# filrg/attackFL

Hardware: AMD Instinct MI355X
Metric: FL rounds/sec (whole node) + test-acc, TransformerModel/ICU, 8 clients (higher is better)
Workload: dtype bf16; 1 GPU; model=TransformerModel, global_batch=1024, seq_len=1, parallelism=fl8-clients-over-1-ranks, clients=8, local_epochs=5, rows_per_client=12000-15000, mode=fedavg, trainer=fused

## Files before the change

csrc/kernels/tf2.hip:

```cpp
#include "common.h"
#include "kernels.h"
#include "tf_common.h"
#include "fused_common.h"
#include "onchip.h"

using namespace tf;

namespace t2 {

using namespace oc;



constexpr int LDDN = 24 * 2, LDVO = LD64 + 16;
constexpr int B_IMG_D = 0;
constexpr int B_IMG_V = B_IMG_D + 64 * LDDN;
constexpr int B_IMG_O = B_IMG_V + 64 * LDVO;
constexpr int B_IMG_F1 = B_IMG_O + 64 * LDVO;
constexpr int B_IMG_F2 = B_IMG_F1 + 16 * LD64;
constexpr int B_H0 = B_IMG_F2 + 64 * LD32;
constexpr int B_A = B_H0 + 16384;
constexpr int B_X1N = B_A + 16384;
constexpr int B_DF3 = B_X1N + 16384;
constexpr int B_DO = B_DF3 + 16384;
constexpr int B_DV = B_DO + 16384;
constexpr int B_DZ0 = B_DV + 16384;
constexpr int B_XIN = B_DZ0 + 16384;
constexpr int B_F2 = B_XIN + 4096;
constexpr int B_DF0 = B_F2 + 4096;
constexpr int B_NVEC = 648;
constexpr int B_VEC = B_DF0 + 4096;
constexpr int B_CS = B_VEC + B_NVEC * 4;
constexpr int B_NLN = 6 * 64;
constexpr int B_DBL = B_CS;
constexpr int B_DBL_BYTES = B_NLN * 8;
static_assert(B_DBL_BYTES >= B_NVEC * 4, "DBL covers CS");
constexpr int B_MISC = B_DBL + B_DBL_BYTES;
constexpr int B_CNT_A = B_MISC + 32;
constexpr int B_CNT_B = B_MISC + 36;
constexpr int B_CNT_C = B_MISC + 40;
constexpr int B_TOTAL = B_MISC + 64;
enum { VS_DB = 0, VS_VB, VS_OB, VS_G1, VS_B1, VS_F2B, VS_G2, VS_B2, VS_G3, VS_B3 };
constexpr int VS_F1B = 640;

#ifndef TF2_HLD1
#define TF2_HLD1 (LD128 + 16)
#endif
#ifndef TF2_HLD2
#define TF2_HLD2 (LD64 + 16)
#endif
constexpr int HLD1 = TF2_HLD1, HLD2 = TF2_HLD2;
constexpr int H_IMG_W1 = 0;
constexpr int H_IMG_W2 = H_IMG_W1 + 64 * HLD1;
constexpr int H_CAT = H_IMG_W2 + 32 * HLD2;
constexpr int H_A1 = H_CAT + 32768;
constexpr int H_DZ1 = H_A1 + 16384;
constexpr int H_DZ2 = H_DZ1 + 16384;
constexpr int H_NVEC = 132;
constexpr int H_VEC = H_DZ2 + 8192;
constexpr int H_PART = H_VEC + H_NVEC * 4;
constexpr int H_LOSS = H_PART + 8 * H_NVEC * 4;
constexpr int H_TOTAL = H_LOSS + 64;
enum { HV_B1 = 0, HV_B2 = 64, HV_WO = 96, HV_BO = 128 };

constexpr int SMEM_CORE = B_TOTAL > H_TOTAL ? B_TOTAL : H_TOTAL;
#ifdef TF2_STAMPS
constexpr int ST_OFF = SMEM_CORE, ST_N = 16;
constexpr int SMEM = ST_OFF + ST_N * 8;
#else
constexpr int SMEM = SMEM_CORE;
#endif
static_assert(SMEM <= 160 * 1024, "LDS budget");

constexpr int MOM_SLOTS = 11;
constexpr long WS_MOM = 0;
constexpr long MOM_WG_BYTES = (long)MOM_SLOTS * NTH * 16;
constexpr int CMP_SLOTS = 1;
constexpr long BR_UNITS = (long)CMP_SLOTS * NTH * 16;
constexpr long BR_SMALL = BR_UNITS + 8L * 12 * 64 * 16;
constexpr long BR_WG_BYTES = BR_SMALL + 4L * 9 * 64 * 16;
constexpr long WS_BYTES = WS_MOM + MOM_WG_BYTES + 2 * BR_WG_BYTES;

__device__ __forceinline__ void ln_colsum(uchar* smem, int k, const float (&x)[16], int lane) {
  float s;
  const int f = colsum64(x, lane, s);
  lds_addq(smem + B_DBL, 64 * k + f, s);
}
__host__ __device__ constexpr int ln_seg(int k) { return k < 2 ? VS_G1 + k : VS_G2 + (k - 2); }
static_assert(ln_seg(0) == VS_G1 && ln_seg(1) == VS_B1 && ln_seg(2) == VS_G2 && ln_seg(3) == VS_B2 &&
              ln_seg(4) == VS_G3 && ln_seg(5) == VS_B3, "DBL order");

__device__ __forceinline__ uint32_t mask16(uint32_t key, uint32_t layer, int r, int g, uint32_t thr) {
  uint32_t m = 0;
#pragma unroll
  for (int t = 0; t < 4; ++t) {
#pragma unroll
    for (int h = 0; h < 2; ++h) {
      const uint32_t x = hash3(key, layer, (uint32_t)r, (uint32_t)(8 * t + 2 * g + h));
      m |= ((x & 0xFFFFu) >= thr ? 1u : 0u) << (4 * t + 2 * h);
      m |= ((x >> 16) >= thr ? 1u : 0u) << (4 * t + 2 * h + 1);
    }
  }
  return m;
}


#ifdef TF2_STAMPS
struct Stamp {
  bool on = false;
  int who = 0;
  uchar* smem = nullptr;
  __device__ __forceinline__ void operator()(int id, int tid) {
    if (!on) return;
    const uint64_t now = __builtin_amdgcn_s_memrealtime();
    if (tid == who) {
      LDS_AS uint64_t* t = (LDS_AS uint64_t*)(smem + ST_OFF);
      t[id] += now - t[ST_N - 1];
      t[ST_N - 1] = now;
    }
  }
};
#else
struct Stamp {
  __device__ __forceinline__ void operator()(int, int) {}
};
#endif

enum { ABL_U3 = 1, ABL_UADAM = 2, ABL_UDW = 4, ABL_COLSUM = 8, ABL_HEADUPD = 16, ABL_U1 = 32 };
#if defined(TF2_STAMPS) && defined(TF2_ABL)
#define ABL(K, b) ((TF2_ABL & (b)) != 0)
#else
#define ABL(K, b) false
#endif



#ifndef TF2_NO_PRIO
__device__ __forceinline__ void prio_hi() { __builtin_amdgcn_s_setprio(2); }
__device__ __forceinline__ void prio_lo() { __builtin_amdgcn_s_setprio(0); }
#else
__device__ __forceinline__ void prio_hi() {}
__device__ __forceinline__ void prio_lo() {}
#endif

template <int BR>
struct BrK {
  static constexpr BrOff o = BR == 0 ? OV : OL;
  static constexpr int din = BR == 0 ? D_V : D_L;
  static constexpr int xoff = BR == 0 ? 0 : D_V;
  static constexpr Mat MV{o.inproj_w + 128 * 64, 64, 64, B_IMG_V, LDVO};
  static constexpr Mat MO{o.out_w, 64, 64, B_IMG_O, LDVO};
  static __device__ __forceinline__ Mat vo(bool lo) {
    return Mat{lo ? MV.off : MO.off, 64, 64, lo ? B_IMG_V : B_IMG_O, LDVO};
  }
  static __device__ __forceinline__ int vec_param(int e) {
    if (e >= VS_F1B) return e - VS_F1B < FF ? o.ff0_b + (e - VS_F1B) : -1;
    const int s = e >> 6, i = e & 63;
    const int b = s == 0 ? o.dense_b : s == 1 ? o.inproj_b + 128 : s == 2 ? o.out_b : s == 3 ? o.ln1_w
                : s == 4 ? o.ln1_b : s == 5 ? o.ff3_b : s == 6 ? o.ln2_w : s == 7 ? o.ln2_b : s == 8 ? o.bn_w : o.bn_b;
    return b + i;
  }
};

struct Saved {
  uint32_t xh1[8], xh2[8], gp[8];
  float rstd1, rstd2;
  uint32_t m1, m2, matt;
  float gk[4];
};
__device__ __forceinline__ void save16(uint32_t (&d)[8], const float (&x)[16]) {
#pragma unroll
  for (int k = 0; k < 8; ++k) d[k] = pk2(x[2 * k], x[2 * k + 1]);
}
__device__ __forceinline__ void load16(float (&x)[16], const uint32_t (&d)[8]) {
#pragma unroll
  for (int k = 0; k < 8; ++k) {
    x[2 * k] = __uint_as_float(d[k] << 16);
    x[2 * k + 1] = __uint_as_float(d[k] & 0xFFFF0000u);
  }
}

constexpr int NCMP = 2;
struct BrState {
  VS cmp[NCMP];
  float dst[NCMP];
};
static_assert(B_NVEC <= NCMP * NTH, "compact entries");

template <int BR>
__device__ __forceinline__ void br_masks(uint32_t key, int r, int g, uint32_t& mk0, uint32_t& mk1) {
  const uint32_t ha = hash3(key, 8 * BR + L_ATT, r, 0), hb = hash3(key, 8 * BR + L_ATT, r, 1);
  const uint32_t matt = ((ha & 0xFFFFu) >= THR_P01 ? 1u : 0u) | ((ha >> 16) >= THR_P01 ? 2u : 0u) |
                        ((hb & 0xFFFFu) >= THR_P01 ? 4u : 0u) | ((hb >> 16) >= THR_P01 ? 8u : 0u);
  const uint32_t m1 = mask16(key, 8 * BR + L_D1, r, g, THR_P01), m2 = mask16(key, 8 * BR + L_D2, r, g, THR_P01);
  uint32_t kf = 0u;
  if (g < 2) {
    const uint32_t hd[2] = {hash3(key, 8 * BR + L_DF, r, 2 * g), hash3(key, 8 * BR + L_DF, r, 2 * g + 1)};
#pragma unroll
    for (int i = 0; i < 4; ++i) {
      const uint32_t u = (hd[i >> 1] >> ((i & 1) << 4)) & 0xFFFFu;
      kf |= (4 * g + i < FF && u >= THR_P01 ? 1u : 0u) << i;
    }
  }
  mk0 = m1 | (m2 << 16);
  mk1 = matt | (kf << 4);
}

template <int BR>
__device__ __forceinline__ void br_forward(uchar* smem, const float (&xin)[4], uint32_t mk0, uint32_t mk1, Saved& sv,
                                           u32x4 (&outp)[2], int lane, int wave) {
  using B = BrK<BR>;
  opq(lane, wave);
  const int g = lane >> 4, r = 16 * wave + (lane & 15);
  const uchar* vg = lane_vec(smem + B_VEC, g);
  st4<TK16>(smem + B_XIN, r, g, xin);
  float h0[16];
  sb();
  {
    const s4v bx = bfrag4(xin);
    f4v acc[4];
#pragma unroll
    for (int T = 0; T < 4; ++T)
      acc[T] = mma16(*(const LDS_AS s4v*)(smem + B_IMG_D + (16 * T + (lane & 15)) * LDDN + 8 * (lane >> 4)), bx, Z4);
    float bd[16], gp[16];
    vec16g(bd, vg + VS_DB * 256);
#pragma unroll
    for (int t = 0; t < 4; ++t)
#pragma unroll
      for (int i = 0; i < 4; i += 2) {
        gf2v g2;
        const gf2v y = gelu2(gf2v{acc[t][i] + bd[4 * t + i], acc[t][i + 1] + bd[4 * t + i + 1]}, g2);
        h0[4 * t + i] = y[0];
        h0[4 * t + i + 1] = y[1];
        gp[4 * t + i] = g2[0];
        gp[4 * t + i + 1] = g2[1];
      }
    save16(sv.gp, gp);
#pragma unroll
    for (int t = 0; t < 4; ++t) st4<TK64>(smem + B_H0, r, 4 * t + g, h0 + 4 * t);
  }
  float a[16];
  sb();
  {
    const s8v b0 = bfrag(h0, 0), b1 = bfrag(h0, 1);
    f4v acc[4];
#pragma unroll
    for (int T = 0; T < 4; ++T) {
      acc[T] = mma(wfrag(smem + B_IMG_V, LDVO, T, 0, lane), b0, Z4);
      acc[T] = mma(wfrag(smem + B_IMG_V, LDVO, T, 1, lane), b1, acc[T]);
    }
    sv.matt = mk1 & 0xFu;
    float bv[16];
    vec16g(bv, vg + VS_VB * 256);
#pragma unroll
    for (int t = 0; t < 4; ++t) {
      const float m = keepf(INV_K01, sv.matt, t);
#pragma unroll
      for (int i = 0; i < 4; ++i) a[4 * t + i] = (acc[t][i] + bv[4 * t + i]) * m;
    }
#pragma unroll
    for (int t = 0; t < 4; ++t) st4<TK64>(smem + B_A, r, 4 * t + g, a + 4 * t);
  }
  float x1n[16];
  sb();
  {
    const s8v b0 = bfrag(a, 0), b1 = bfrag(a, 1);
    f4v acc[4];
#pragma unroll
    for (int T = 0; T < 4; ++T) {
      acc[T] = mma(wfrag(smem + B_IMG_O, LDVO, T, 0, lane), b0, Z4);
      acc[T] = mma(wfrag(smem + B_IMG_O, LDVO, T, 1, lane), b1, acc[T]);
    }
    sv.m1 = mk0 & 0xFFFFu;
    float bo[16];
    vec16g(bo, vg + VS_OB * 256);
    float x1[16];
#pragma unroll
    for (int t = 0; t < 4; ++t)
#pragma unroll
      for (int i = 0; i < 4; ++i) {
        const int j = 4 * t + i;
        x1[j] = h0[j] + keepf((acc[t][i] + bo[j]) * INV_K01, sv.m1, j);
      }
    sv.rstd1 = ln_fwd2(x1);
    save16(sv.xh1, x1);
    float gm[16], bt[16];
    vec16g(gm, vg + VS_G1 * 256);
    vec16g(bt, vg + VS_B1 * 256);
    affine2(x1n, x1, gm, bt);
#pragma unroll
    for (int t = 0; t < 4; ++t) st4<TK64>(smem + B_X1N, r, 4 * t + g, x1n + 4 * t);
  }
  float f2v[4];
  sb();
  {
    f4v acc = mma(wfrag(smem + B_IMG_F1, LD64, 0, 0, lane), bfrag(x1n, 0), Z4);
    acc = mma(wfrag(smem + B_IMG_F1, LD64, 0, 1, lane), bfrag(x1n, 1), acc);
    const f4v bf = g < 2 ? *(const LDS_AS f4v*)(vg + VS_F1B * 4) : Z4;
#pragma unroll
    for (int i = 0; i < 4; ++i) {
      float gp;
      const float gl = gelu_and_grad(acc[i] + bf[i], gp);
      f2v[i] = keepf(gl * INV_K01, mk1, 4 + i);
      sv.gk[i] = keepf(gp * INV_K01, mk1, 4 + i);
    }
    st4<TK16>(smem + B_F2, r, g, f2v);
  }
  sb();
  {
    const s4v bf = bfrag4(f2v);
    f4v acc[4];
#pragma unroll
    for (int T = 0; T < 4; ++T) acc[T] = mma16(wfrag4(smem + B_IMG_F2, LD32, T, lane), bf, Z4);
    sv.m2 = mk0 >> 16;
    float b3[16];
    vec16g(b3, vg + VS_F2B * 256);
    float x2[16];
#pragma unroll
    for (int t = 0; t < 4; ++t)
#pragma unroll
      for (int i = 0; i < 4; ++i) {
        const int j = 4 * t + i;
        x2[j] = x1n[j] + keepf((acc[t][i] + b3[j]) * INV_K01, sv.m2, j);
      }
    sv.rstd2 = ln_fwd2(x2);
    save16(sv.xh2, x2);
    float gm[16], bt[16];
    vec16g(gm, vg + VS_G2 * 256);
    vec16g(bt, vg + VS_B2 * 256);
    affine2(x2, x2, gm, bt);
    ln_fwd2(x2);
    vec16g(gm, vg + VS_G3 * 256);
    vec16g(bt, vg + VS_B3 * 256);
    affine2(x2, x2, gm, bt);
    pack16(x2, outp);
  }
}

template <int BR>
__device__ __forceinline__ void br_backward(uchar* smem, const float (&dout)[16], const Saved& sv, const AdamK& K, int lane,
                                            int wave) {
  opq(lane, wave);
  const int g = lane >> 4, r = 16 * wave + (lane & 15);
  const uchar* vg = lane_vec(smem + B_VEC, g);
  float dr2[16];
  sb();
  {
    float gm[16], t[16], dx[16], xh[16], bt[16];
    load16(xh, sv.xh2);
    vec16g(gm, vg + VS_G2 * 256);
    vec16g(bt, vg + VS_B2 * 256);
    affine2(xh, xh, gm, bt);
    const float rstd3 = ln_fwd2(xh);
#pragma unroll
    for (int j = 0; j < 16; ++j) t[j] = dout[j] * xh[j];
    if (!ABL(K, ABL_COLSUM)) ln_colsum(smem, 4, t, lane);
    if (!ABL(K, ABL_COLSUM)) ln_colsum(smem, 5, dout, lane);
    vec16g(gm, vg + VS_G3 * 256);
    ln_bwd2(dx, dout, xh, rstd3, gm);
    load16(xh, sv.xh2);
#pragma unroll
    for (int j = 0; j < 16; ++j) t[j] = dx[j] * xh[j];
    if (!ABL(K, ABL_COLSUM)) ln_colsum(smem, 2, t, lane);
    if (!ABL(K, ABL_COLSUM)) ln_colsum(smem, 3, dx, lane);
    vec16g(gm, vg + VS_G2 * 256);
    ln_bwd2(dr2, dx, xh, sv.rstd2, gm);
  }
  float df0[4];
  sb();
  {
    float d3[16];
#pragma unroll
    for (int j = 0; j < 16; ++j) d3[j] = keepf(dr2[j] * INV_K01, sv.m2, j);
#pragma unroll
    for (int t = 0; t < 4; ++t) st4<TK64>(smem + B_DF3, r, 4 * t + g, d3 + 4 * t);
    f4v acc = mma(wtfrag<true>(smem + B_IMG_F2, LD32, 0, 0, lane), bfrag(d3, 0), Z4);
    acc = mma(wtfrag<true>(smem + B_IMG_F2, LD32, 0, 1, lane), bfrag(d3, 1), acc);
#pragma unroll
    for (int i = 0; i < 4; ++i) df0[i] = acc[i] * sv.gk[i];
    st4<TK16>(smem + B_DF0, r, g, df0);
  }
  lds_signal(smem, B_CNT_C, lane);
  float dr1[16];
  sb();
  {
    const s4v bd = bfrag4(df0);
    float dx[16];
#pragma unroll
    for (int T = 0; T < 4; ++T) {
      const f4v acc = mma16(wtfrag4(smem + B_IMG_F1, LD64, T, lane), bd, Z4);
#pragma unroll
      for (int i = 0; i < 4; ++i) dx[4 * T + i] = acc[i] + dr2[4 * T + i];
    }
    float t[16], gm[16], xh[16];
    load16(xh, sv.xh1);
#pragma unroll
    for (int j = 0; j < 16; ++j) t[j] = dx[j] * xh[j];
    if (!ABL(K, ABL_COLSUM)) ln_colsum(smem, 0, t, lane);
    if (!ABL(K, ABL_COLSUM)) ln_colsum(smem, 1, dx, lane);
    vec16g(gm, vg + VS_G1 * 256);
    ln_bwd2(dr1, dx, xh, sv.rstd1, gm);
  }
  float dv[16];
  sb();
  {
    float dO[16];
#pragma unroll
    for (int j = 0; j < 16; ++j) dO[j] = keepf(dr1[j] * INV_K01, sv.m1, j);
#pragma unroll
    for (int t = 0; t < 4; ++t) st4<TK64>(smem + B_DO, r, 4 * t + g, dO + 4 * t);
    const s8v b0 = bfrag(dO, 0), b1 = bfrag(dO, 1);
#pragma unroll
    for (int T = 0; T < 4; ++T) {
      f4v acc = mma(wtfrag<true>(smem + B_IMG_O, LDVO, T, 0, lane), b0, Z4);
      acc = mma(wtfrag<true>(smem + B_IMG_O, LDVO, T, 1, lane), b1, acc);
      const float m = keepf(INV_K01, sv.matt, T);
#pragma unroll
      for (int i = 0; i < 4; ++i) dv[4 * T + i] = acc[i] * m;
    }
#pragma unroll
    for (int t = 0; t < 4; ++t) st4<TK64>(smem + B_DV, r, 4 * t + g, dv + 4 * t);
  }
  lds_signal(smem, B_CNT_A, lane);
  sb();
  {
    const s8v b0 = bfrag(dv, 0), b1 = bfrag(dv, 1);
    float dz[16], gp[16];
    load16(gp, sv.gp);
#pragma unroll
    for (int T = 0; T < 4; ++T) {
      f4v acc = mma(wtfrag<true>(smem + B_IMG_V, LDVO, T, 0, lane), b0, Z4);
      acc = mma(wtfrag<true>(smem + B_IMG_V, LDVO, T, 1, lane), b1, acc);
#pragma unroll
      for (int i = 0; i < 4; ++i) dz[4 * T + i] = (acc[i] + dr1[4 * T + i]) * gp[4 * T + i];
    }
#pragma unroll
    for (int t = 0; t < 4; ++t) st4<TK64>(smem + B_DZ0, r, 4 * t + g, dz + 4 * t);
  }
  lds_signal(smem, B_CNT_B, lane);
}


template <int BR>
__device__ __forceinline__ int cmp_param(int e) {
  return e < B_NVEC ? BrK<BR>::vec_param(e) : -1;
}
template <int BR>
__device__ __forceinline__ uint32_t cmp_dst(int e, int lane) {
  const uint32_t dmy = B_DF0 + 768 + 4 * lane;
  return cmp_param<BR>(e) >= 0 ? (0x80000000u | (uint32_t)(B_VEC + 4 * e)) : (0x80000000u | dmy);
}

__device__ __forceinline__ f4v unit_ld(__amdgpu_buffer_rsrc_t rm, int ui, int j, int lane) {
  return __builtin_bit_cast(f4v, __builtin_amdgcn_raw_buffer_load_b128(rm, (int)BR_UNITS + ((ui * 12 + j) * 64 + lane) * 16,
                                                                        0, 16));
}
__device__ __forceinline__ void unit_st(__amdgpu_buffer_rsrc_t rm, int ui, int j, int lane, f4v v) {
  __builtin_amdgcn_raw_buffer_store_b128(__builtin_bit_cast(u32x4, v), rm, (int)BR_UNITS + ((ui * 12 + j) * 64 + lane) * 16,
                                         0, 0);
  store_guard();
}
__device__ __forceinline__ void unit_adam(f4v (&U)[12], const f4v (&acc)[2][2], const AdamK& K) {
  float p[16], mm[16], vv[16], g[16], den[16];
#pragma unroll
  for (int t = 0; t < 4; ++t)
#pragma unroll
    for (int i = 0; i < 4; ++i) {
      mm[4 * t + i] = U[t][i];
      vv[4 * t + i] = U[4 + t][i];
      p[4 * t + i] = U[8 + t][i];
      g[4 * t + i] = acc[t >> 1][t & 1][i];
    }
#pragma unroll
  for (int e = 0; e < 16; ++e) {
    const float mk = mm[e] * K.keep;
    mm[e] = mk + K.c1 * (g[e] - mk);
    vv[e] = fk::B2 * vv[e] + (1.f - fk::B2) * g[e] * g[e];
  }
#pragma unroll
  for (int e = 0; e < 16; ++e) den[e] = __builtin_amdgcn_sqrtf(vv[e]);
#pragma unroll
  for (int e = 0; e < 16; ++e) den[e] = __builtin_amdgcn_rcpf(den[e] * K.rsqrt_bc2 + K.eps);
#pragma unroll
  for (int e = 0; e < 16; ++e) p[e] -= K.lr_bc1 * mm[e] * den[e];
#pragma unroll
  for (int t = 0; t < 4; ++t)
#pragma unroll
    for (int i = 0; i < 4; ++i) {
      U[t][i] = mm[4 * t + i];
      U[4 + t][i] = vv[4 * t + i];
      U[8 + t][i] = p[4 * t + i];
    }
}
__device__ __forceinline__ void unit_img(uchar* smem, const Mat& M, int Ta, int Tb, int lane, const u32x2v (&w)[4]) {
  const int i16 = lane & 15, g4 = 4 * (lane >> 4);
#pragma unroll
  for (int t = 0; t < 4; ++t)
    *(LDS_AS u32x2v*)(smem + M.img + (16 * (Tb + (t & 1)) + i16) * M.ld + pcol(16 * (Ta + (t >> 1)) + g4) * 2) = w[t];
}
__device__ __forceinline__ void unit_pack(const f4v (&U)[12], u32x2v (&w)[4]) {
#pragma unroll
  for (int t = 0; t < 4; ++t) w[t] = u32x2v{pk2(U[8 + t][0], U[8 + t][1]), pk2(U[8 + t][2], U[8 + t][3])};
}
__device__ __forceinline__ void unit_dw(const uchar* X, const uchar* DY, int Ta, int Tb, int lane, bool bias,
                                        f4v (&acc)[2][2], f4v (&bs)[2]) {
#pragma unroll
  for (int a = 0; a < 2; ++a)
#pragma unroll
    for (int b = 0; b < 2; ++b) acc[a][b] = Z4;
  bs[0] = bs[1] = Z4;
  uint32_t o1 = 0x3F803F80u;
  asm volatile("" : "+s"(o1));
  const s8v one = __builtin_bit_cast(s8v, u32x4{o1, o1, o1, o1});
#pragma unroll
  for (int s = 0; s < 4; ++s) {
    const s8v x0 = tfrag<TK64>(X, 32 * s, Ta, lane), x1 = tfrag<TK64>(X, 32 * s, Ta + 1, lane);
    const s8v y0 = tfrag<TK64>(DY, 32 * s, Tb, lane), y1 = tfrag<TK64>(DY, 32 * s, Tb + 1, lane);
    acc[0][0] = mma(x0, y0, acc[0][0]);
    acc[0][1] = mma(x0, y1, acc[0][1]);
    acc[1][0] = mma(x1, y0, acc[1][0]);
    acc[1][1] = mma(x1, y1, acc[1][1]);
    if (bias) {
      bs[0] = mma(one, y0, bs[0]);
      bs[1] = mma(one, y1, bs[1]);
    }
  }
}

__device__ __forceinline__ f4v smu_ld(__amdgpu_buffer_rsrc_t rm, int w4, int j, int lane) {
  return __builtin_bit_cast(f4v, __builtin_amdgcn_raw_buffer_load_b128(rm, (int)BR_SMALL + ((w4 * 9 + j) * 64 + lane) * 16,
                                                                        0, 16));
}
__device__ __forceinline__ void smu_st(__amdgpu_buffer_rsrc_t rm, int w4, int j, int lane, f4v v) {
  __builtin_amdgcn_raw_buffer_store_b128(__builtin_bit_cast(u32x4, v), rm, (int)BR_SMALL + ((w4 * 9 + j) * 64 + lane) * 16,
                                         0, 0);
  store_guard();
}
template <int BR>
__device__ __forceinline__ void smu_elem(int s, int w4, int lane, int i, int& pi, int& img) {
  using B = BrK<BR>;
  constexpr int din = BrK<BR>::din;
  const int g = lane >> 4, i16 = lane & 15;
  if (s == 0) {
    const int n = 16 * w4 + i16, k = 4 * g + i;
    pi = k < din ? B::o.dense_w + n * din + k : -1;
    img = B_IMG_D + n * LDDN + k * 2;
  } else if (s == 1) {
    const int n = 16 * w4 + i16, k = 4 * g + i;
    pi = k < FF ? B::o.ff3_w + n * FF + k : -1;
    img = B_IMG_F2 + n * LD32 + pcol(k) * 2;
  } else {
    const int n = i16, k = 16 * w4 + 4 * g + i;
    pi = n < FF ? B::o.ff0_w + n * 64 + k : -1;
    img = B_IMG_F1 + n * LD64 + pcol(k) * 2;
  }
}
__device__ __forceinline__ void smu_adam(f4v (&S)[9], const f4v (&gs)[3], const AdamK& K) {
  float p[12], mm[12], vv[12], g[12], den[12];
#pragma unroll
  for (int s = 0; s < 3; ++s)
#pragma unroll
    for (int i = 0; i < 4; ++i) {
      mm[4 * s + i] = S[s][i];
      vv[4 * s + i] = S[3 + s][i];
      p[4 * s + i] = S[6 + s][i];
      g[4 * s + i] = gs[s][i];
    }
#pragma unroll
  for (int e = 0; e < 12; ++e) {
    const float mk = mm[e] * K.keep;
    mm[e] = mk + K.c1 * (g[e] - mk);
    vv[e] = fk::B2 * vv[e] + (1.f - fk::B2) * g[e] * g[e];
  }
#pragma unroll
  for (int e = 0; e < 12; ++e) den[e] = __builtin_amdgcn_sqrtf(vv[e]);
#pragma unroll
  for (int e = 0; e < 12; ++e) den[e] = __builtin_amdgcn_rcpf(den[e] * K.rsqrt_bc2 + K.eps);
#pragma unroll
  for (int e = 0; e < 12; ++e) p[e] -= K.lr_bc1 * mm[e] * den[e];
#pragma unroll
  for (int s = 0; s < 3; ++s)
#pragma unroll
    for (int i = 0; i < 4; ++i) {
      S[s][i] = mm[4 * s + i];
      S[3 + s][i] = vv[4 * s + i];
      S[6 + s][i] = p[4 * s + i];
    }
}
template <int BR>
__device__ __forceinline__ void smu_img(uchar* smem, const f4v (&S)[9], int w4, int lane) {
#pragma unroll
  for (int s = 0; s < 3; ++s) {
    int pi, img;
    smu_elem<BR>(s, w4, lane, 0, pi, img);
    *(LDS_AS u32x2v*)(smem + img) = u32x2v{pk2(S[6 + s][0], S[6 + s][1]), pk2(S[6 + s][2], S[6 + s][3])};
  }
}

template <int BR>
__device__ __forceinline__ bool br_update(uchar* smem, BrState& st, const AdamK& K, int lane, int wave, int tid, int step,
                                          __amdgpu_buffer_rsrc_t rm, Stamp& stp, gu32* tmo) {
  using B = BrK<BR>;
  opq(lane, wave);
  asm volatile("" : "+v"(tid));
  const int w4 = wave & 3, g = lane >> 4, i16 = lane & 15;
  const bool lead = wave < 4;
  const uint32_t all = 8u * (uint32_t)step;
  LDS_AS uint32_t* abort_w = ldsu(smem, B_MISC);
  const int Ta = 2 * (w4 & 1), Tb = 2 * (w4 >> 1);
  const bool do_bias = (w4 & 1) == 0;
  f4v bsu[2];
  f4v as = Z4, bd = Z4, a3 = Z4, af1 = Z4, b3 = Z4, b1 = Z4;
  const int ui = 2 * w4 + (lead ? 0 : 1);
  f4v U[12];
#pragma unroll
  for (int j = 0; j < 12; ++j) U[j] = unit_ld(rm, ui, j, lane);
  uint32_t o1 = 0x3F803F80u;
  asm volatile("" : "+s"(o1));
  const s8v one = __builtin_bit_cast(s8v, u32x4{o1, o1, o1, o1});
  if (lead) {
    prio_lo();
    if (!lds_wait(smem, B_CNT_C, all)) {
      if (lane == 0) __hip_atomic_store(tmo, 1u, __ATOMIC_RELAXED, __HIP_MEMORY_SCOPE_AGENT);
      return false;
    }
#pragma unroll
    for (int s = 0; s < (ABL(K, ABL_U1) ? 0 : 4); ++s) {
      const s8v y3 = tfrag<TK64>(smem + B_DF3, 32 * s, w4, lane), y1 = tfrag<TK16>(smem + B_DF0, 32 * s, 0, lane);
      a3 = mma(tfrag<TK16>(smem + B_F2, 32 * s, 0, lane), y3, a3);
      af1 = mma(tfrag<TK64>(smem + B_X1N, 32 * s, w4, lane), y1, af1);
      b3 = mma(one, y3, b3);
      if (wave == 0) b1 = mma(one, y1, b1);
    }
    if (!lds_wait(smem, B_CNT_A, all)) {
      if (lane == 0) __hip_atomic_store(tmo, 1u, __ATOMIC_RELAXED, __HIP_MEMORY_SCOPE_AGENT);
      return false;
    }
    prio_hi();
  } else {
    if (!lds_wait(smem, B_CNT_A, all)) {
      if (lane == 0) __hip_atomic_store(tmo, 1u, __ATOMIC_RELAXED, __HIP_MEMORY_SCOPE_AGENT);
      return false;
    }
  }
  {
    uint32_t any = 0;
#pragma unroll
    for (int i = 0; i < 8; ++i) any |= abort_w[i];
    if (any) return false;
  }
  stp(4, tid);
  {
    f4v acc[2][2];
    if (!ABL(K, ABL_UDW))
      unit_dw(smem + (lead ? B_A : B_H0), smem + (lead ? B_DO : B_DV), Ta, Tb, lane, do_bias, acc, bsu);
    if (!ABL(K, ABL_UADAM)) unit_adam(U, acc, K);
    u32x2v w[4];
    unit_pack(U, w);
    if (!lead && !lds_wait(smem, B_CNT_B, all)) {
      if (lane == 0) __hip_atomic_store(tmo, 1u, __ATOMIC_RELAXED, __HIP_MEMORY_SCOPE_AGENT);
      return false;
    }
    unit_img(smem, B::vo(!lead), Ta, Tb, lane, w);
#pragma unroll
    for (int j = 0; j < 12; ++j) unit_st(rm, ui, j, lane, U[j]);
  }
  if (lead) {
    f4v S[9];
#pragma unroll
    for (int j = 0; j < 9; ++j) S[j] = smu_ld(rm, w4, j, lane);
    if (!lds_wait(smem, B_CNT_B, all)) {
      if (lane == 0) __hip_atomic_store(tmo, 1u, __ATOMIC_RELAXED, __HIP_MEMORY_SCOPE_AGENT);
      return false;
    }
#pragma unroll
    for (int s = 0; s < (ABL(K, ABL_U1) ? 0 : 4); ++s) {
      const s8v yd = tfrag<TK64>(smem + B_DZ0, 32 * s, w4, lane);
      as = mma(tfrag<TK16>(smem + B_XIN, 32 * s, 0, lane), yd, as);
      bd = mma(one, yd, bd);
    }
    const f4v gs3[3] = {as, a3, af1};
    if (!ABL(K, ABL_U3)) smu_adam(S, gs3, K);
    smu_img<BR>(smem, S, w4, lane);
#pragma unroll
    for (int j = 0; j < 9; ++j) smu_st(rm, w4, j, lane, S[j]);
  }
  const float lnsum = tid < B_NLN ? lds_getq(smem + B_DBL, tid) : 0.f;
  const f4v cmom = mom_ld(rm, 0, tid);
  stp(5, tid);
  prio_hi();
  lds_bar();
  {
    LDS_AS float* cs = ldsf(smem, B_CS);
    if (tid < B_NLN) cs[ln_seg(tid >> 6) * 64 + (tid & 63)] = lnsum;
    if (do_bias && g == 0) {
#pragma unroll
      for (int b = 0; b < 2; ++b) cs[(lead ? VS_OB : VS_VB) * 64 + 16 * (Tb + b) + i16] = bsu[b][0];
    }
    if (lead) {
      if (g == 0) {
        cs[VS_F2B * 64 + 16 * w4 + i16] = b3[0];
        cs[VS_DB * 64 + 16 * w4 + i16] = bd[0];
        if (wave == 0 && i16 < FF) cs[VS_F1B + i16] = b1[0];
      }
    }
  }
  lds_bar();
  stp(6, tid);
  if (tid < (B_DBL_BYTES - B_NVEC * 4) / 4) ldsf(smem, B_CS)[B_NVEC + tid] = 0.f;
  float mm[NCMP] = {cmom[0], cmom[1]}, vv[NCMP] = {cmom[2], cmom[3]};
  if (!ABL(K, ABL_U3)) {
    const int dmy = B_DF0 + 4 * (tid & 63);
    float gr[NCMP], pn[NCMP];
#pragma unroll
    for (int h = 0; h < NCMP; ++h) {
      const int e = tid + NTH * h;
      gr[h] = e < B_NVEC ? *(const LDS_AS float*)(smem + B_CS + 4 * e) : 0.f;
    }
    adam_staged<NCMP>(st.cmp, mm, vv, gr, pn, K);
#pragma unroll
    for (int h = 0; h < NCMP; ++h) {
      const int e = tid + NTH * h;
      const uint32_t d = aru(st.dst[h]);
      const bool vec = e < B_NVEC;
      const bool f32 = d >> 31;
      const int off = (int)(d & 0x7FFFFFFFu);
      *(LDS_AS float*)(smem + (vec ? B_CS + 4 * e : dmy)) = 0.f;
      *(LDS_AS float*)(smem + (f32 ? off : dmy + 256)) = pn[h];
      *(LDS_AS unsigned short*)(smem + (f32 ? dmy + 512 : off)) = fk::f2bf(pn[h]);
    }
  }
  mom_st(rm, 0, tid, f4v{mm[0], mm[1], vv[0], vv[1]});
  return true;
}

__device__ __forceinline__ void mom_zero(__amdgpu_buffer_rsrc_t rm, int tid) {
#pragma unroll
  for (int k = 0; k < MOM_SLOTS; ++k) mom_st(rm, k, tid, Z4);
}

template <int BR>
__device__ __forceinline__ void br_init(uchar* smem, BrState& st, const float* P, __amdgpu_buffer_rsrc_t rm, int lane,
                                        int wave, int tid) {
  using B = BrK<BR>;
#pragma unroll
  for (int k = 0; k < CMP_SLOTS; ++k) mom_st(rm, k, tid, Z4);
  {
    const int w4 = wave & 3, u = wave >> 2, Ta = 2 * (w4 & 1), Tb = 2 * (w4 >> 1);
    const Mat M = B::vo(u == 1);
    const int i16 = lane & 15, g4 = 4 * (lane >> 4);
#pragma unroll
    for (int t = 0; t < 4; ++t) {
      const int n = 16 * (Tb + (t & 1)) + i16, k0 = 16 * (Ta + (t >> 1)) + g4;
      const float* src = P + M.off + n * M.k_real + k0;
      const f4v p = {src[0], src[1], src[2], src[3]};
      unit_st(rm, 2 * w4 + u, t, lane, Z4);
      unit_st(rm, 2 * w4 + u, 4 + t, lane, Z4);
      unit_st(rm, 2 * w4 + u, 8 + t, lane, p);
      *(LDS_AS u32x2v*)(smem + M.img + n * M.ld + pcol(k0) * 2) = u32x2v{pk2(p[0], p[1]), pk2(p[2], p[3])};
    }
  }
  if (wave < 4) {
    f4v S[9];
#pragma unroll
    for (int s = 0; s < 3; ++s) {
      S[s] = S[3 + s] = Z4;
#pragma unroll
      for (int i = 0; i < 4; ++i) {
        int pi, img;
        smu_elem<BR>(s, wave, lane, i, pi, img);
        S[6 + s][i] = pi >= 0 ? P[pi] : 0.f;
      }
    }
    smu_img<BR>(smem, S, wave, lane);
#pragma unroll
    for (int j = 0; j < 9; ++j) smu_st(rm, wave, j, lane, S[j]);
  }
#pragma unroll
  for (int h = 0; h < NCMP; ++h) {
    const int e = tid + NTH * h;
    float p0 = 0.f;
    if (e < B_NVEC) {
      const int pi = cmp_param<BR>(e);
      p0 = pi >= 0 ? P[pi] : 0.f;
      ldsf(smem, B_VEC)[e] = p0;
      ldsf(smem, B_CS)[e] = 0.f;
    }
    st.cmp[h] = VS{aw(p0)};
    st.dst[h] = awu(cmp_dst<BR>(e, lane));
  }
}

template <int BR>
__device__ __forceinline__ void br_fini(const BrState& st, float* P, __amdgpu_buffer_rsrc_t rm, int lane, int wave,
                                        int tid) {
  using B = BrK<BR>;
  {
    asm volatile("s_waitcnt vmcnt(0)" ::: "memory");
    __syncthreads();
    const int w4 = wave & 3, u = wave >> 2, Ta = 2 * (w4 & 1), Tb = 2 * (w4 >> 1);
    const Mat M = B::vo(u == 1);
    const int i16 = lane & 15, g4 = 4 * (lane >> 4);
#pragma unroll
    for (int t = 0; t < 4; ++t) {
      const int n = 16 * (Tb + (t & 1)) + i16, k0 = 16 * (Ta + (t >> 1)) + g4;
      const f4v p = unit_ld(rm, 2 * w4 + u, 8 + t, lane);
      float* dst = P + M.off + n * M.k_real + k0;
#pragma unroll
      for (int i = 0; i < 4; ++i) dst[i] = p[i];
      store_guard();
    }
  }
  if (wave < 4) {
#pragma unroll
    for (int s = 0; s < 3; ++s) {
      const f4v p = smu_ld(rm, wave, 6 + s, lane);
#pragma unroll
      for (int i = 0; i < 4; ++i) {
        int pi, img;
        smu_elem<BR>(s, wave, lane, i, pi, img);
        if (pi >= 0) P[pi] = p[i];
      }
      store_guard();
    }
  }
#pragma unroll
  for (int h = 0; h < NCMP; ++h) {
    const int e = tid + NTH * h;
    if (e < B_NVEC) {
      const int pi = cmp_param<BR>(e);
      if (pi >= 0) P[pi] = ar(st.cmp[h].p);
    }
  }
}

template <int BR>
__device__ __forceinline__ void load_x(float (&x)[4], const AflTfTrainArgs& a, int cid, const Walk& w, int r, int g) {
  const int Bn = min(a.batch, a.nd[cid] - w.b0);
  const gi32* ord = (const gi32*)(a.order + ((long)cid * a.E + w.e) * a.maxnd);
  const bool valid = r < Bn;
  const int ridx = valid ? ord[w.b0 + r] : 0;
  const gf* row = (const gf*)a.rows + (long)ridx * ROW + BrK<BR>::xoff;
#pragma unroll
  for (int i = 0; i < 4; ++i) {
    const int c = 4 * g + i;
    x[i] = (valid && c < BrK<BR>::din) ? row[c] : 0.f;
  }
}

__device__ __forceinline__ void stamp_init(Stamp& stp, const AflTfTrainArgs& a, uchar* smem) {
#ifdef TF2_STAMPS
  stp.on = a.stamps && (long)blockIdx.x == (long)a.stamps[63];
  stp.who = a.stamps ? 64 * (int)(a.stamps[62] & 7) : 0;
  stp.smem = smem;
  if (threadIdx.x == 0) *(LDS_AS uint64_t*)(smem + ST_OFF + 8 * (ST_N - 1)) = __builtin_amdgcn_s_memrealtime();
#endif
  (void)stp; (void)a; (void)smem;
}
__device__ __forceinline__ void stamp_fini(Stamp& stp, const AflTfTrainArgs& a, uchar* smem, int tid) {
#ifdef TF2_STAMPS
  if (stp.on && tid == 0)
    for (int i = 0; i < ST_N - 1; ++i) a.stamps[i] = *(LDS_AS uint64_t*)(smem + ST_OFF + 8 * i);
#endif
  (void)stp; (void)a; (void)smem; (void)tid;
}

template <int BR>
__device__ __forceinline__ void branch_main(const AflTfTrainArgs& a, int cid, uchar* smem) {
  const int tid = threadIdx.x, lane = tid & 63, wave = __builtin_amdgcn_readfirstlane(tid >> 6), g = lane >> 4;
  float* P = a.params + (long)cid * NPARAM;
  uchar* ws = (uchar*)(a.ws + (long)cid * a.ws_stride);
  gu32* sync = (gu32*)(a.sync + (long)cid * AFL_TF2_SYNC_WORDS);
  const __amdgpu_buffer_rsrc_t rg = gr_rsrc(sync);
  for (int i = tid; i < SMEM / 4; i += NTH) ldsf(smem, 0)[i] = 0.f;
  __syncthreads();
  BrState st;
  const __amdgpu_buffer_rsrc_t rm = rsrc(ws + WS_MOM + MOM_WG_BYTES + BR * BR_WG_BYTES);
  br_init<BR>(smem, st, P, rm, lane, wave, tid);
  asm volatile("s_waitcnt vmcnt(0)" ::: "memory");
  __syncthreads();
  Stamp stp;
  stamp_init(stp, a, smem);

  const int nd = a.nd[cid], BS = a.batch, E = a.E;
  const uint32_t seed = a.seeds[cid];
  LDS_AS uint32_t* abort_w = ldsu(smem, B_MISC);
  int step = 0;
  bool failed = false;
  Walk w{0, 0};
  float xin[4];
  bool more = walk_valid(w, nd, BS, E);
  if (more) load_x<BR>(xin, a, cid, w, 16 * wave + (lane & 15), g);
  float mka0, mka1;
  {
    uint32_t m0, m1;
    br_masks<BR>(afl_hash32(seed, 1u), 16 * wave + (lane & 15), g, m0, m1);
    mka0 = awu(m0);
    mka1 = awu(m1);
  }
  while (more) {
    ++step;
    const AdamK K = adam_k(a, step);
    Saved sv;
    u32x4 outp[2];
    prio_hi();
    asm volatile(";MARK fwd");
#ifndef TF2_NO_FWD
    br_forward<BR>(smem, xin, aru(mka0), aru(mka1), sv, outp, lane, wave);
#else
    sv = Saved{}; outp[0] = u32x4{0,0,0,0}; outp[1] = outp[0];
#endif
    asm volatile(";MARK fwd_end");
    stp(0, tid);
    gr_put(rg, gr_off(0, BR, wave, lane), outp, (uint32_t)step);
    prio_lo();
    w.b0 += BS;
    more = walk_valid(w, nd, BS, E);
    if (more) load_x<BR>(xin, a, cid, w, 16 * wave + (lane & 15), g);
    {
      uint32_t m0, m1;
      br_masks<BR>(afl_hash32(seed, (uint32_t)(step + 1)), 16 * wave + (lane & 15), g, m0, m1);
      mka0 = awu(m0);
      mka1 = awu(m1);
    }
    stp(1, tid);
    u32x4 du[2];
    const int go[1] = {gr_off(1, BR, wave, lane)};
    const uint32_t fv = gr_get<1>(rg, go, du, (uint32_t)step, 1, sync + XF_TMO, lane);
    prio_hi();
    stp(2, tid);
    if (fv == 0xFFFFFFFFu) {
      if (lane == 0) abort_w[wave] = 1u;
      lds_signal(smem, B_CNT_A, lane);
      lds_signal(smem, B_CNT_B, lane);
      failed = true;
      break;
    }
    float dout[16];
    unpack16(du, dout);
    if (lane == 0) abort_w[wave] = fv & 1u;
#ifndef TF2_NO_BWD
    asm volatile(";MARK bwd");
    br_backward<BR>(smem, dout, sv, K, lane, wave);
    asm volatile(";MARK bwd_end");
    stp(3, tid);
#else
    for (int j = 0; j < 16; ++j) asm volatile("" :: "v"(dout[j]));
    lds_signal(smem, B_CNT_A, lane);
    lds_signal(smem, B_CNT_B, lane);
#endif
    asm volatile(";MARK upd");
    const bool upd_ok = br_update<BR>(smem, st, K, lane, wave, tid, step, rm, stp, sync + XF_TMO);
    asm volatile(";MARK upd_end");
    if (!upd_ok) {
      failed = true;
      break;
    }
    stp(7, tid);
    lds_bar();
    stp(8, tid);
  }
  (void)failed;
  stamp_fini(stp, a, smem, tid);
  br_fini<BR>(st, P, rm, lane, wave, tid);
}

constexpr Mat HW1{FC1_W, 64, 128, H_IMG_W1, HLD1};
constexpr Mat HW2{FC2_W, 32, 64, H_IMG_W2, HLD2};
__device__ __forceinline__ int hvec_param(int e) {
  return e < 64 ? FC1_B + e : e < 96 ? FC2_B + (e - 64) : e < 128 ? OUT_W + (e - 96) : e == 128 ? OUT_B : -1;
}
struct HdState {
  TS blk[4];
  TS t2;
  VS vec;
};

__device__ __forceinline__ void head_main(const AflTfTrainArgs& a, int cid, uchar* smem) {
  const int tid = threadIdx.x, lane = tid & 63, wave = __builtin_amdgcn_readfirstlane(tid >> 6), g = lane >> 4;
  const int r = 16 * wave + (lane & 15);
  float* P = a.params + (long)cid * NPARAM;
  uchar* ws = (uchar*)(a.ws + (long)cid * a.ws_stride);
  gu32* sync = (gu32*)(a.sync + (long)cid * AFL_TF2_SYNC_WORDS);
  const __amdgpu_buffer_rsrc_t rg = gr_rsrc(sync);
  for (int i = tid; i < SMEM / 4; i += NTH) ldsf(smem, 0)[i] = 0.f;
  __syncthreads();
  HdState st;
  Stamp stp;
  const __amdgpu_buffer_rsrc_t rm = rsrc(ws + WS_MOM);
  mom_zero(rm, tid);
  {
    const int Ta = 2 * (wave & 3), Tb = 2 * (wave >> 2);
#pragma unroll
    for (int x = 0; x < 2; ++x)
#pragma unroll
      for (int y = 0; y < 2; ++y) tile_load(st.blk[2 * x + y], HW1, Ta + x, Tb + y, lane, P, smem);
    tile_load(st.t2, HW2, wave & 3, wave >> 2, lane, P, smem);
    float p0 = 0.f;
    if (tid < H_NVEC) {
      const int pi = hvec_param(tid);
      p0 = pi >= 0 ? P[pi] : 0.f;
      ldsf(smem, H_VEC)[tid] = p0;
    }
    st.vec = VS{aw(p0)};
  }
  __syncthreads();
  stamp_init(stp, a, smem);

  const int nd = a.nd[cid], BS = a.batch, E = a.E;
  const int nb_total = (nd + BS - 1) / BS;
  const uint32_t seed = a.seeds[cid];
  const uchar* vec = smem + H_VEC;
  LDS_AS float* part = ldsf(smem, H_PART) + wave * H_NVEC;
  LDS_AS float* lossw = ldsf(smem, H_LOSS);
  int step = 0;
  bool failed = false, timed_out = false;
  float epoch_loss = 0.f;
  Walk w{0, 0};
  int cur_e = 0;
  bool more = walk_valid(w, nd, BS, E);
  float lab = 0.f;
  auto load_lab = [&](const Walk& ww) {
    const int Bn = min(BS, nd - ww.b0);
    const gi32* ord = (const gi32*)(a.order + ((long)cid * E + ww.e) * a.maxnd);
    lab = r < Bn ? ((const gf*)a.rows)[(long)ord[ww.b0 + r] * ROW + ROW - 1] : 0.f;
  };
  if (more) load_lab(w);
  while (more) {
    while (cur_e < w.e) {
      if (tid == 0) a.losses[(long)cid * E + cur_e] = epoch_loss / (float)max(nb_total, 1);
      epoch_loss = 0.f;
      ++cur_e;
    }
    ++step;
    const AdamK K = adam_k(a, step);
    const uint32_t key = afl_hash32(seed, (uint32_t)step);
    const int Bn = min(BS, nd - w.b0);
    const bool valid = r < Bn;
    const float inv_bn = 1.f / (float)Bn;
    const uint32_t mh = mask16(key, L_HEAD, r, g, THR_P03);
    sb();
    u32x4 cv[4];
    const int go[2] = {gr_off(0, 0, wave, lane), gr_off(0, 1, wave, lane)};
    const uint32_t fv = gr_get<2>(rg, go, cv, (uint32_t)step, 0, sync + XF_TMO, lane);
    if (fv == 0xFFFFFFFFu) {
      timed_out = failed = true;
      break;
    }
    prio_hi();
    stp(10, tid);
    float a1[16], gk1[16];
    {
      f4v acc[4];
#pragma unroll
      for (int T = 0; T < 4; ++T) {
        acc[T] = Z4;
#pragma unroll
        for (int s = 0; s < 4; ++s)
          acc[T] = mma(wfrag(smem + H_IMG_W1, HLD1, T, s, lane), __builtin_bit_cast(s8v, cv[s]), acc[T]);
      }
      float b1[16];
      vec16(b1, vec + HV_B1 * 4, g);
#pragma unroll
      for (int t = 0; t < 4; ++t)
#pragma unroll
        for (int i = 0; i < 4; i += 2) {
          const int j = 4 * t + i;
          gf2v gp;
          const gf2v gl = gelu2(gf2v{acc[t][i] + b1[j], acc[t][i + 1] + b1[j + 1]}, gp);
#pragma unroll
          for (int h = 0; h < 2; ++h) {
            a1[j + h] = keepf(gl[h] * INV_K03, mh, j + h);
            gk1[j + h] = keepf(gp[h] * INV_K03, mh, j + h);
          }
        }
    }
    float dz2[8], gw[8];
    float dy3 = 0.f, pl = 0.f;
    {
      const s8v b0 = bfrag(a1, 0), b1 = bfrag(a1, 1);
      f4v acc[2];
#pragma unroll
      for (int T = 0; T < 2; ++T) {
        acc[T] = mma(wfrag(smem + H_IMG_W2, HLD2, T, 0, lane), b0, Z4);
        acc[T] = mma(wfrag(smem + H_IMG_W2, HLD2, T, 1, lane), b1, acc[T]);
      }
      float b2[8], wo[8], g2[8], gp2[8];
      vec8(b2, vec + HV_B2 * 4, g);
      vec8(wo, vec + HV_WO * 4, g);
      float dot = 0.f;
#pragma unroll
      for (int t = 0; t < 2; ++t)
#pragma unroll
        for (int i = 0; i < 4; i += 2) {
          const int j = 4 * t + i;
          gf2v gp;
          const gf2v gl = gelu2(gf2v{acc[t][i] + b2[j], acc[t][i + 1] + b2[j + 1]}, gp);
          g2[j] = gl[0];
          g2[j + 1] = gl[1];
          gp2[j] = gp[0];
// ... 265 lines not shown
```

Baseline: 118.3 rounds/s.

## Remove compact-staging LDS barriers in vector Adam and precompute backward LN prologue

Replaces the staged compact-vector Adam update, which went through an LDS staging area and two block barriers, with a per-thread fixed mapping (vec_entry). Each thread now takes its bias and LN-colsum gradient straight from registers or the double accumulator and writes the updated parameter directly. The backward LN3 recomputation and the F2 weight fragments are hoisted ahead of the cross-branch gradient exchange wait, and the momentum load is issued earlier, so this latency overlaps the wait. It also adds missing CNT_C signals on abort paths. In exchange it raises register pressure and relies on a hand-derived ownership mapping being correct.

```diff
diff --git a/csrc/kernels/tf2.hip b/csrc/kernels/tf2.hip
--- a/csrc/kernels/tf2.hip
+++ b/csrc/kernels/tf2.hip
@@ -30,11 +30,9 @@
 constexpr int B_DF0 = B_F2 + 4096;
 constexpr int B_NVEC = 648;
 constexpr int B_VEC = B_DF0 + 4096;
-constexpr int B_CS = B_VEC + B_NVEC * 4;
 constexpr int B_NLN = 6 * 64;
-constexpr int B_DBL = B_CS;
+constexpr int B_DBL = B_VEC + B_NVEC * 4;
 constexpr int B_DBL_BYTES = B_NLN * 8;
-static_assert(B_DBL_BYTES >= B_NVEC * 4, "DBL covers CS");
 constexpr int B_MISC = B_DBL + B_DBL_BYTES;
 constexpr int B_CNT_A = B_MISC + 32;
 constexpr int B_CNT_B = B_MISC + 36;
@@ -183,9 +181,18 @@
 constexpr int NCMP = 2;
 struct BrState {
   VS cmp[NCMP];
-  float dst[NCMP];
 };
-static_assert(B_NVEC <= NCMP * NTH, "compact entries");
+__device__ __forceinline__ int vec_entry(int wave, int lane, int h) {
+  const int w4 = wave & 3, g = lane >> 4, i16 = lane & 15;
+  const bool lead = wave < 4;
+  if (h == 0) {
+    if (wave >= 2) return ln_seg(wave - 2) * 64 + lane;
+    return wave == 0 && g == 0 && VS_F1B + i16 < B_NVEC ? VS_F1B + i16 : -1;
+  }
+  if (g < 2) return (w4 & 1) == 0 ? (lead ? VS_OB : VS_VB) * 64 + 16 * (2 * (w4 >> 1) + g) + i16 : -1;
+  return lead ? (g == 2 ? VS_F2B : VS_DB) * 64 + 16 * w4 + i16 : -1;
+}
+__device__ __forceinline__ bool vec_real(int e) { return e >= 0 && e < VS_F1B + FF; }
 
 template <int BR>
 __device__ __forceinline__ void br_masks(uint32_t key, int r, int g, uint32_t& mk0, uint32_t& mk1) {
@@ -337,21 +344,39 @@
   }
 }
 
+struct BwdPre {
+  float xh3[16], rstd3;
+  s8v f3[2];
+};
+__device__ __forceinline__ void br_bwd_pre(const uchar* smem, const Saved& sv, BwdPre& bp, int lane) {
+  const uchar* vg = lane_vec(smem + B_VEC, lane >> 4);
+  float gm[16], bt[16];
+  load16(bp.xh3, sv.xh2);
+  vec16g(gm, vg + VS_G2 * 256);
+  vec16g(bt, vg + VS_B2 * 256);
+  affine2(bp.xh3, bp.xh3, gm, bt);
+  bp.rstd3 = ln_fwd2(bp.xh3);
+#pragma unroll
+  for (int j = 0; j < 16; ++j) asm volatile("" : "+v"(bp.xh3[j]));
+  asm volatile("" : "+v"(bp.rstd3));
+  bp.f3[0] = wtfrag<true>(smem + B_IMG_F2, LD32, 0, 0, lane);
+  bp.f3[1] = wtfrag<true>(smem + B_IMG_F2, LD32, 0, 1, lane);
+  asm volatile("" : "+v"(bp.f3[0]), "+v"(bp.f3[1]));
+}
+
 template <int BR>
-__device__ __forceinline__ void br_backward(uchar* smem, const float (&dout)[16], const Saved& sv, const AdamK& K, int lane,
-                                            int wave) {
+__device__ __forceinline__ void br_backward(uchar* smem, const float (&dout)[16], const Saved& sv, const BwdPre& bp,
+                                            const AdamK& K, int lane, int wave) {
   opq(lane, wave);
   const int g = lane >> 4, r = 16 * wave + (lane & 15);
   const uchar* vg = lane_vec(smem + B_VEC, g);
   float dr2[16];
   sb();
   {
-    float gm[16], t[16], dx[16], xh[16], bt[16];
-    load16(xh, sv.xh2);
-    vec16g(gm, vg + VS_G2 * 256);
-    vec16g(bt, vg + VS_B2 * 256);
-    affine2(xh, xh, gm, bt);
-    const float rstd3 = ln_fwd2(xh);
+    float gm[16], t[16], dx[16], xh[16];
+#pragma unroll
+    for (int j = 0; j < 16; ++j) xh[j] = bp.xh3[j];
+    const float rstd3 = bp.rstd3;
 #pragma unroll
     for (int j = 0; j < 16; ++j) t[j] = dout[j] * xh[j];
     if (!ABL(K, ABL_COLSUM)) ln_colsum(smem, 4, t, lane);
@@ -374,8 +399,8 @@
     for (int j = 0; j < 16; ++j) d3[j] = keepf(dr2[j] * INV_K01, sv.m2, j);
 #pragma unroll
     for (int t = 0; t < 4; ++t) st4<TK64>(smem + B_DF3, r, 4 * t + g, d3 + 4 * t);
-    f4v acc = mma(wtfrag<true>(smem + B_IMG_F2, LD32, 0, 0, lane), bfrag(d3, 0), Z4);
-    acc = mma(wtfrag<true>(smem + B_IMG_F2, LD32, 0, 1, lane), bfrag(d3, 1), acc);
+    f4v acc = mma(bp.f3[0], bfrag(d3, 0), Z4);
+    acc = mma(bp.f3[1], bfrag(d3, 1), acc);
 #pragma unroll
     for (int i = 0; i < 4; ++i) df0[i] = acc[i] * sv.gk[i];
     st4<TK16>(smem + B_DF0, r, g, df0);
@@ -443,12 +468,7 @@
 
 template <int BR>
 __device__ __forceinline__ int cmp_param(int e) {
-  return e < B_NVEC ? BrK<BR>::vec_param(e) : -1;
-}
-template <int BR>
-__device__ __forceinline__ uint32_t cmp_dst(int e, int lane) {
-  const uint32_t dmy = B_DF0 + 768 + 4 * lane;
-  return cmp_param<BR>(e) >= 0 ? (0x80000000u | (uint32_t)(B_VEC + 4 * e)) : (0x80000000u | dmy);
+  return vec_real(e) ? BrK<BR>::vec_param(e) : -1;
 }
 
 __device__ __forceinline__ f4v unit_ld(__amdgpu_buffer_rsrc_t rm, int ui, int j, int lane) {
@@ -597,19 +617,45 @@
   }
 }
 
+template <int N>
+__device__ __forceinline__ void vec_adam(VS (&pa)[N], float (&m)[N], float (&v)[N], const float (&g)[N], float (&pn)[N],
+                                         const AdamK& K) {
+#pragma clang fp contract(off)
+  float den[N];
+#pragma unroll
+  for (int i = 0; i < N; ++i) {
+    pn[i] = ar(pa[i].p);
+    const float mk = m[i] * K.keep;
+    m[i] = __builtin_fmaf(K.c1, g[i] - mk, mk);
+    const float t = (1.f - fk::B2) * g[i], u = fk::B2 * v[i];
+    v[i] = __builtin_fmaf(g[i], t, u);
+  }
+#pragma unroll
+  for (int i = 0; i < N; ++i) den[i] = __builtin_amdgcn_sqrtf(v[i]);
+#pragma unroll
+  for (int i = 0; i < N; ++i) den[i] = __builtin_amdgcn_rcpf(__builtin_fmaf(K.rsqrt_bc2, den[i], K.eps));
+#pragma unroll
+  for (int i = 0; i < N; ++i) {
+    const float lm = K.lr_bc1 * m[i];
+    pn[i] = __builtin_fmaf(-lm, den[i], pn[i]);
+    pa[i].p = aw(pn[i]);
+  }
+}
+
 template <int BR>
 __device__ __forceinline__ bool br_update(uchar* smem, BrState& st, const AdamK& K, int lane, int wave, int tid, int step,
                                           __amdgpu_buffer_rsrc_t rm, Stamp& stp, gu32* tmo) {
   using B = BrK<BR>;
   opq(lane, wave);
   asm volatile("" : "+v"(tid));
-  const int w4 = wave & 3, g = lane >> 4, i16 = lane & 15;
+  const int w4 = wave & 3, g = lane >> 4;
   const bool lead = wave < 4;
   const uint32_t all = 8u * (uint32_t)step;
   LDS_AS uint32_t* abort_w = ldsu(smem, B_MISC);
   const int Ta = 2 * (w4 & 1), Tb = 2 * (w4 >> 1);
   const bool do_bias = (w4 & 1) == 0;
-  f4v bsu[2];
+  f4v bsu[2] = {Z4, Z4};
+  f4v cmom;
   f4v as = Z4, bd = Z4, a3 = Z4, af1 = Z4, b3 = Z4, b1 = Z4;
   const int ui = 2 * w4 + (lead ? 0 : 1);
   f4v U[12];
@@ -657,6 +703,7 @@
     if (!ABL(K, ABL_UADAM)) unit_adam(U, acc, K);
     u32x2v w[4];
     unit_pack(U, w);
+    cmom = mom_ld(rm, 0, tid);
     if (!lead && !lds_wait(smem, B_CNT_B, all)) {
       if (lane == 0) __hip_atomic_store(tmo, 1u, __ATOMIC_RELAXED, __HIP_MEMORY_SCOPE_AGENT);
       return false;
@@ -685,49 +732,24 @@
 #pragma unroll
     for (int j = 0; j < 9; ++j) smu_st(rm, w4, j, lane, S[j]);
   }
-  const float lnsum = tid < B_NLN ? lds_getq(smem + B_DBL, tid) : 0.f;
-  const f4v cmom = mom_ld(rm, 0, tid);
   stp(5, tid);
   prio_hi();
-  lds_bar();
-  {
-    LDS_AS float* cs = ldsf(smem, B_CS);
-    if (tid < B_NLN) cs[ln_seg(tid >> 6) * 64 + (tid & 63)] = lnsum;
-    if (do_bias && g == 0) {
-#pragma unroll
-      for (int b = 0; b < 2; ++b) cs[(lead ? VS_OB : VS_VB) * 64 + 16 * (Tb + b) + i16] = bsu[b][0];
-    }
-    if (lead) {
-      if (g == 0) {
-        cs[VS_F2B * 64 + 16 * w4 + i16] = b3[0];
-        cs[VS_DB * 64 + 16 * w4 + i16] = bd[0];
-        if (wave == 0 && i16 < FF) cs[VS_F1B + i16] = b1[0];
-      }
-    }
-  }
-  lds_bar();
-  stp(6, tid);
-  if (tid < (B_DBL_BYTES - B_NVEC * 4) / 4) ldsf(smem, B_CS)[B_NVEC + tid] = 0.f;
+  float gr[NCMP];
+  gr[0] = b1[0];
+  if (wave >= 2) {
+    LDS_AS double* q = (LDS_AS double*)(smem + B_DBL) + 64 * (wave - 2) + lane;
+    gr[0] = lds_getq(smem + B_DBL, 64 * (wave - 2) + lane);
+    *q = 0.0;
+  }
+  gr[1] = g == 0 ? bsu[0][0] : g == 1 ? bsu[1][0] : g == 2 ? b3[0] : bd[0];
   float mm[NCMP] = {cmom[0], cmom[1]}, vv[NCMP] = {cmom[2], cmom[3]};
   if (!ABL(K, ABL_U3)) {
-    const int dmy = B_DF0 + 4 * (tid & 63);
-    float gr[NCMP], pn[NCMP];
+    float pn[NCMP];
+    vec_adam<NCMP>(st.cmp, mm, vv, gr, pn, K);
 #pragma unroll
     for (int h = 0; h < NCMP; ++h) {
-      const int e = tid + NTH * h;
-      gr[h] = e < B_NVEC ? *(const LDS_AS float*)(smem + B_CS + 4 * e) : 0.f;
-    }
-    adam_staged<NCMP>(st.cmp, mm, vv, gr, pn, K);
-#pragma unroll
-    for (int h = 0; h < NCMP; ++h) {
-      const int e = tid + NTH * h;
-      const uint32_t d = aru(st.dst[h]);
-      const bool vec = e < B_NVEC;
-      const bool f32 = d >> 31;
-      const int off = (int)(d & 0x7FFFFFFFu);
-      *(LDS_AS float*)(smem + (vec ? B_CS + 4 * e : dmy)) = 0.f;
-      *(LDS_AS float*)(smem + (f32 ? off : dmy + 256)) = pn[h];
-      *(LDS_AS unsigned short*)(smem + (f32 ? dmy + 512 : off)) = fk::f2bf(pn[h]);
+      const int e = vec_entry(wave, lane, h);
+      if (vec_real(e)) ldsf(smem, B_VEC)[e] = pn[h];
     }
   }
   mom_st(rm, 0, tid, f4v{mm[0], mm[1], vv[0], vv[1]});
@@ -778,16 +800,14 @@
   }
 #pragma unroll
   for (int h = 0; h < NCMP; ++h) {
-    const int e = tid + NTH * h;
+    const int e = vec_entry(wave, lane, h);
     float p0 = 0.f;
-    if (e < B_NVEC) {
+    if (e >= 0) {
       const int pi = cmp_param<BR>(e);
       p0 = pi >= 0 ? P[pi] : 0.f;
       ldsf(smem, B_VEC)[e] = p0;
-      ldsf(smem, B_CS)[e] = 0.f;
     }
     st.cmp[h] = VS{aw(p0)};
-    st.dst[h] = awu(cmp_dst<BR>(e, lane));
   }
 }
 
@@ -795,6 +815,7 @@
 __device__ __forceinline__ void br_fini(const BrState& st, float* P, __amdgpu_buffer_rsrc_t rm, int lane, int wave,
                                         int tid) {
   using B = BrK<BR>;
+  opq(lane, wave);
   {
     asm volatile("s_waitcnt vmcnt(0)" ::: "memory");
     __syncthreads();
@@ -826,8 +847,8 @@
   }
 #pragma unroll
   for (int h = 0; h < NCMP; ++h) {
-    const int e = tid + NTH * h;
-    if (e < B_NVEC) {
+    const int e = vec_entry(wave, lane, h);
+    if (e >= 0) {
       const int pi = cmp_param<BR>(e);
       if (pi >= 0) P[pi] = ar(st.cmp[h].p);
     }
@@ -923,6 +944,10 @@
       mka0 = awu(m0);
       mka1 = awu(m1);
     }
+    BwdPre bp;
+    sb();
+    br_bwd_pre(smem, sv, bp, lane);
+    sb();
     stp(1, tid);
     u32x4 du[2];
     const int go[1] = {gr_off(1, BR, wave, lane)};
@@ -931,6 +956,7 @@
     stp(2, tid);
     if (fv == 0xFFFFFFFFu) {
       if (lane == 0) abort_w[wave] = 1u;
+      lds_signal(smem, B_CNT_C, lane);
       lds_signal(smem, B_CNT_A, lane);
       lds_signal(smem, B_CNT_B, lane);
       failed = true;
@@ -941,11 +967,12 @@
     if (lane == 0) abort_w[wave] = fv & 1u;
 #ifndef TF2_NO_BWD
     asm volatile(";MARK bwd");
-    br_backward<BR>(smem, dout, sv, K, lane, wave);
+    br_backward<BR>(smem, dout, sv, bp, K, lane, wave);
     asm volatile(";MARK bwd_end");
     stp(3, tid);
 #else
     for (int j = 0; j < 16; ++j) asm volatile("" :: "v"(dout[j]));
+    lds_signal(smem, B_CNT_C, lane);
     lds_signal(smem, B_CNT_A, lane);
     lds_signal(smem, B_CNT_B, lane);
 #endif
```

After: 123.0 rounds/s, median of 6. 1.04x the previous value.
